# kfjahnke/envutil

Hardware: AMD Instinct MI355X
Metric: Mpix/s reprojected (16K lat/lon->cubemap, b-spline-3) (higher is better)
Workload: dtype f32

## Files before the change

### envutil_amd/csrc/eu_render4.hip

```cpp
#include <cstdio>
#include <cstring>
#include <vector>
#include <algorithm>
#include "eu_packed_dev.h"
#include "eu_launch.h"

#define EU4_TW 16
#define EU4_TH 8
#define EU4_WAVES 4
#ifndef EU4_WAVES0
#define EU4_WAVES0 1
#define EU4_TEXELS 384
#define EU4_OCC0 4
#endif
#define EU4_UNIT_ROWS 4
#define EU4_COL_FLOATS 8
#define EU4_MAX_PLANS 16

__device__ __forceinline__ void eu4_box_reduce(int &mn0, int &mn1, int &mx0, int &mx1)
{
#define EU4_RED(ctrl)                                        \
  "v_min_i32_dpp %0, %0, %0 " ctrl "\n\t"                    \
  "v_min_i32_dpp %1, %1, %1 " ctrl "\n\t"                    \
  "v_max_i32_dpp %2, %2, %2 " ctrl "\n\t"                    \
// ... 325 lines not shown
#pragma unroll 1
  for (int k = gid / EU4_SHARDS; k < nwork; k += (int)(gridDim.x * EU4_WAVES / EU4_SHARDS)) {
    const int id = __builtin_amdgcn_readfirstlane(p.wl[EU4_WL_ENTRIES + (size_t)k * EU4_SHARDS + sh]);
    const int tile_y = id / w.tiles16;
    const int x0 = (id - tile_y * w.tiles16) * EU4_TW;
    eu4_direct_tile<NCH, DEG, PRJ>(p, atab, tile_y, x0, lane);
  }
  __shared__ int last, listed;
  __syncthreads();
  if (threadIdx.x == 0) { listed = 0; last = atomicAdd(p.wl + EU4_WL_DONE1, 1) == (int)gridDim.x - 1; }
  __syncthreads();
  if (last) {
    int mine = 0;
    for (int i = threadIdx.x; i < EU4_SHARDS; i += 256)
      mine += __hip_atomic_load(p.wl + EU4_WL_SHARD(i), __ATOMIC_RELAXED, __HIP_MEMORY_SCOPE_AGENT);
    atomicAdd(&listed, mine);
    for (int i = threadIdx.x; i <= EU4_SHARDS + 8; i += 256)
      __hip_atomic_store(p.wl + 16 * i, 0, __ATOMIC_RELAXED, __HIP_MEMORY_SCOPE_AGENT);
    __syncthreads();
    if (threadIdx.x == 0) __hip_atomic_store(p.wl + EU4_WL_LISTED, listed, __ATOMIC_RELAXED, __HIP_MEMORY_SCOPE_AGENT);
  }
}

static long long eu4_followers_plan = 0, eu4_followers_last = 0;
extern "C" unsigned long long eu_hip_share_follower_tiles(void) { return (unsigned long long)eu4_followers_last; }
static int eu4_boxtab_last = 0;
static long long eu4_boxtab_tiles_last = 0;
extern "C" int eu_hip_boxtab_used(void) { return eu4_boxtab_last; }
extern "C" unsigned long long eu_hip_boxtab_tiles(void) { return (unsigned long long)eu4_boxtab_tiles_last; }

#ifndef EU4_DIRECT_WGS
#define EU4_DIRECT_WGS 2048
#endif

template <int NCH, int DEG, int PRJ>
static int launch4_ndp(const eu_render_params &p, const eu4_plan &w, hipStream_t st)
{
  if constexpr (PRJ == EU_SPHERICAL) {
    static const int cus = [] {
      int dev = 0, n = 0;
      if (hipGetDevice(&dev) != hipSuccess) return 0;
      if (hipDeviceGetAttribute(&n, hipDeviceAttributeMultiprocessorCount, dev) != hipSuccess) return 0;
      return n;
    }();
    const bool fast = eu_staged_fast_profile(p);
    const bool bt = fast && w.boxtab != nullptr && p.out_stride < (1ll << 25);
    int per_cu = 0;
    if (bt) {
      static const int occ = [] { int n = 0; return hipOccupancyMaxActiveBlocksPerMultiprocessor(&n, eu_render5_kernel<NCH, DEG, PRJ, true, true>, 64 * EU5_WAVES, 0) == hipSuccess ? n : 0; }();
      per_cu = occ;
    } else if (fast) {
      static const int occ = [] { int n = 0; return hipOccupancyMaxActiveBlocksPerMultiprocessor(&n, eu_render5_kernel<NCH, DEG, PRJ, true>, 64 * EU5_WAVES, 0) == hipSuccess ? n : 0; }();
      per_cu = occ;
    } else {
      static const int occ = [] { int n = 0; return hipOccupancyMaxActiveBlocksPerMultiprocessor(&n, eu_render5_kernel<NCH, DEG, PRJ, false>, 64 * EU5_WAVES, 0) == hipSuccess ? n : 0; }();
      per_cu = occ;
    }
    const int wgs = (cus / 8) * 8 * per_cu;
    if (wgs <= 0) return -1;
    if (fast) eu4_followers_last = eu4_followers_plan;
    eu4_boxtab_last = bt;
    if (bt) hipLaunchKernelGGL((eu_render5_kernel<NCH, DEG, PRJ, true, true>), dim3((unsigned)wgs), dim3(64 * EU5_WAVES), 0, st, p, w);
    else if (fast) hipLaunchKernelGGL((eu_render5_kernel<NCH, DEG, PRJ, true>), dim3((unsigned)wgs), dim3(64 * EU5_WAVES), 0, st, p, w);
    else hipLaunchKernelGGL((eu_render5_kernel<NCH, DEG, PRJ, false>), dim3((unsigned)wgs), dim3(64 * EU5_WAVES), 0, st, p, w);
  } else {
    const int units = (p.tiles_y + EU4_UNIT_ROWS - 1) / EU4_UNIT_ROWS;
    dim3 grid((unsigned)(8 * ((w.tiles16 + EU4_WAVES0 - 1) / EU4_WAVES0)), (unsigned)EU4_UNIT_ROWS, (unsigned)((units + 7) / 8));
    hipLaunchKernelGGL((eu_render4s_kernel<NCH, DEG, PRJ>), grid, dim3(64 * EU4_WAVES0), 0, st, p, w);
  }
  if (hipGetLastError() != hipSuccess) return -1;
  hipLaunchKernelGGL((eu_render4d_kernel<NCH, DEG, PRJ>), dim3(EU4_DIRECT_WGS), dim3(256), 0, st, p, w);
  if (hipGetLastError() != hipSuccess) {
    (void)hipMemsetAsync(p.wl, 0, EU4_WL_ENTRIES * sizeof(int), st);
    return -1;
  }
  return 0;
}

template <int NCH, int DEG>
static int launch4_nd(const eu_render_params &p, const eu4_plan &w, hipStream_t st)
{
  switch (p.src.prj) {
    case EU_SPHERICAL: return launch4_ndp<NCH, DEG, EU_SPHERICAL>(p, w, st);
    case EU_CUBEMAP: return launch4_ndp<NCH, DEG, EU_CUBEMAP>(p, w, st);
    case EU_BIATAN6: return launch4_ndp<NCH, DEG, EU_BIATAN6>(p, w, st);
  }
  return -2;
}

template <int NCH>
static int launch4_n(const eu_render_params &p, const eu4_plan &w, hipStream_t st)
{
  switch (p.src.degree) {
    case 1: return launch4_nd<NCH, 1>(p, w, st);
    case 2: return launch4_nd<NCH, 2>(p, w, st);
    case 3: return launch4_nd<NCH, 3>(p, w, st);
  }
  return -2;
}

static_assert(EU_STAGED_TILE_ROWS == EU4_TH && EU_STAGED_MAX_TILES_Y == 65535 * 8 * EU4_UNIT_ROWS, "eu_select.h: eu_staged_covers");
namespace {
struct plan_cache {
  std::vector<unsigned char> key;
  eu_dev_buf<int> tileplan, l2_rows, l1_ent, xtab, boxtab;
  bool has_boxtab = false;
  long long boxtab_tiles = 0;
  eu_dev_buf<float> coltab;
  float *atab = nullptr;
  int planned_rows = 0;
  int l2_off[9] = {};
  int l1_off[9] = {};
  int l1_ecols = 1;
  long long follower_tiles = 0;
  hipStream_t last_stream = nullptr;
} g4s[EU_MAX_SLOTS];
#define g4 (g4s[eu_current_slot()])

bool ensure_atab()
{
  if (g4.atab) return true;
  std::vector<float> tab(768, 0.0f);
  for (int i = 0; i < EU_ATAN_TAB_ENTRIES; i++) eu_atan_tab_entry(i, tab.data() + 8 * i);
  if (hipMalloc((void **)&g4.atab, tab.size() * sizeof(float)) != hipSuccess) return false;
  return hipMemcpy(g4.atab, tab.data(), tab.size() * sizeof(float), hipMemcpyHostToDevice) == hipSuccess;
}

template <int DEG>
void launch_colplan(const eu_render_params &p, float *ct, const float *k, hipStream_t st)
{
  hipLaunchKernelGGL((eu_colplan_kernel<DEG>), dim3((unsigned)((p.width + 511) / 512)), dim3(256), 0, st, p, ct,
                     k[0], k[1], k[2], k[3]);
}

std::vector<unsigned char> eu4_plan_key(const eu_render_params &p, unsigned long long plan_gen, const eu_switches &sw)
{
  std::vector<unsigned char> key(sizeof(unsigned long long) + sizeof(eu_src_dev) + 11 * sizeof(int));
  unsigned char *q = key.data();
  memcpy(q, &plan_gen, sizeof plan_gen); q += sizeof plan_gen;
  eu_src_dev sd = p.src; sd.base = nullptr;
  memcpy(q, &sd, sizeof sd); q += sizeof sd;
  const int v[11] = { p.width, p.row_begin, p.row_end, p.band_shift, p.band_count, p.band_index, p.form, p.norm_mode, sw.share,
                      sw.boxtab, sw.boxtab_max_kb };
  memcpy(q, v, sizeof v);
  return key;
}

bool upload(eu_dev_buf<int> &buf, const std::vector<int> &v, size_t spare)
{
  if (buf.reserve(v.size() + spare) != hipSuccess) return false;
  return v.empty() || hipMemcpy(buf.p, v.data(), v.size() * sizeof(int), hipMemcpyHostToDevice) == hipSuccess;
}

template <int DEG>
void launch_boxplan(const eu_render_params &p, const float *atab_g, const int *l2_rows, int tiles16, int ntiles, int *tab, hipStream_t st)
{
  hipLaunchKernelGGL((eu5_boxplan_kernel<DEG>), dim3((unsigned)((ntiles + 3) / 4)), dim3(256), 0, st, p, atab_g, l2_rows, tiles16,
                     ntiles, tab);
}

int eu4_build_plans(const eu_render_params &p, int tiles16, const eu_switches &sw, const float *h_row,
                    size_t h_row_floats, hipStream_t st)
{
  std::vector<int> tp((size_t)p.tiles_y, -1);
  std::vector<float> plans;
  const bool can = p.form == EU_FORM_BA && p.norm_mode == EU_NORM_NONE && h_row;
// ... 34 lines not shown
    for (int r = 0; r < p.tiles_y; r++)
      if (!paired(r >> 1)) rows[(r / EU5_UNIT_ROWS) & 7].push_back(r);
    for (int x = 0; x < 8; x++) { g4.l2_off[x] = (int)all.size(); all.insert(all.end(), rows[x].begin(), rows[x].end()); }
    g4.l2_off[8] = (int)all.size();
    if (!upload(g4.l2_rows, all, 1)) return -1;
  }
  g4.has_boxtab = false; g4.boxtab_tiles = 0;
  if (sw.boxtab && eu_staged_fast_profile(p)) {
    const long long ntiles = (long long)g4.l2_off[8] * tiles16;
    const long long bytes = ntiles * (EU5_BT_RECS * 16);
    if (bytes <= (long long)sw.boxtab_max_kb * 1024) {
      if (g4.boxtab.reserve((size_t)std::max<long long>(1, ntiles) * (EU5_BT_RECS * 4)) != hipSuccess) return -1;
      if (ntiles > 0) {
        switch (p.src.degree) {
          case 1: launch_boxplan<1>(p, g4.atab, g4.l2_rows.p, tiles16, (int)ntiles, g4.boxtab.p, st); break;
          case 2: launch_boxplan<2>(p, g4.atab, g4.l2_rows.p, tiles16, (int)ntiles, g4.boxtab.p, st); break;
          default: launch_boxplan<3>(p, g4.atab, g4.l2_rows.p, tiles16, (int)ntiles, g4.boxtab.p, st); break;
        }
        if (hipGetLastError() != hipSuccess) return -1;
      }
      g4.has_boxtab = true; g4.boxtab_tiles = ntiles;
    }
  }
  for (int j = 0; j < nplans; j++) {
    float *ct = g4.coltab.p + j * (size_t)p.width * EU4_COL_FLOATS;
    switch (p.src.degree) {
      case 1: launch_colplan<1>(p, ct, &plans[4 * j], st); break;
      case 2: launch_colplan<2>(p, ct, &plans[4 * j], st); break;
      default: launch_colplan<3>(p, ct, &plans[4 * j], st); break;
    }
    if (hipGetLastError() != hipSuccess) return -1;
  }
  std::vector<float> h_ct((size_t)nplans * p.width * EU4_COL_FLOATS);
  if (nplans) {
    if (hipStreamSynchronize(st) != hipSuccess) return -1;
    if (hipMemcpy(h_ct.data(), g4.coltab.p, h_ct.size() * sizeof(float), hipMemcpyDeviceToHost) != hipSuccess) return -1;
  }
  std::vector<int> cm, cp;
  for (int m = 0; 2 * m + 1 < p.tiles_y; m++)
    if (paired(m)) { cm.push_back(m); cp.push_back(tp[(size_t)2 * m]); }
  eu_share_input in;
  in.width = p.width; in.tiles16 = tiles16; in.row_begin = p.row_begin; in.row_end = p.row_end;
  in.band_mode = p.band_count > 1;
  in.ncand = (int)cm.size(); in.cand_m = cm.data(); in.cand_plan = cp.data();
  in.h_row = h_row; in.h_row_floats = h_row_floats; in.row_floats = EU_ROW_FLOATS;
  in.coltab = nplans ? h_ct.data() : nullptr; in.col_floats = EU4_COL_FLOATS; in.nplans = nplans;
// ... 5 lines not shown
  if (hipMemcpy(g4.xtab.p, gr.xtab.data(), gr.xtab.size() * sizeof(int), hipMemcpyHostToDevice) != hipSuccess) return -1;
  for (int x = 0; x < 9; x++) g4.l1_off[x] = gr.off[x];
  g4.l1_ecols = gr.ecols;
  g4.follower_tiles = gr.follower_tiles;
  return 0;
}

void eu4_fill_plan(eu4_plan &w)
{
  w.tileplan = g4.tileplan.p;
  w.coltab = g4.coltab.p;
  w.l2_rows = g4.l2_rows.p;
  for (int x = 0; x < 9; x++) w.l2_off[x] = g4.l2_off[x];
  w.l2_half = (w.tiles16 + 1) / 2;
  w.l2_magic = (1ull << 40) / (unsigned long long)w.l2_half + 1;
  w.l1_ent = g4.l1_ent.p;
  for (int x = 0; x < 9; x++) w.l1_off[x] = g4.l1_off[x];
  w.l1_ecols = g4.l1_ecols;
  w.l1_magic = (1ull << 40) / (unsigned long long)w.l1_ecols + 1;
  w.xtab = g4.xtab.p;
  w.boxtab = g4.has_boxtab ? g4.boxtab.p : nullptr;
}

int launch4(const eu_render_params &p, const eu4_plan &w, hipStream_t st)
{
  switch (p.nch) {
    case 3: return launch4_n<3>(p, w, st);
    case 4: return launch4_n<4>(p, w, st);
  }
  return -2;
}

#ifdef EU5_STAMPS
int launch4_stamped(const eu_render_params &p, eu4_plan &w, hipStream_t st)
{
  static unsigned long long *d_st = nullptr; static size_t st_cap = 0; static int dumps = 0;
  const size_t ntile_st = (size_t)w.tiles16 * p.tiles_y * 8;
  const size_t nst = ntile_st + 8192 * 4;
  if (st_cap < nst) { if (d_st) (void)hipFree(d_st); if (hipMalloc((void **)&d_st, nst * 8) != hipSuccess) return -1; st_cap = nst; }
  (void)hipMemsetAsync(d_st, 0, nst * 8, st);
  w.stamps = d_st;
  const int rc_ = launch4(p, w, st);
  if (rc_ == 0 && dumps < 2 && nst >= 8 * 4096) {
    dumps++;
    std::vector<unsigned long long> h(nst);
    (void)hipStreamSynchronize(st);
    (void)hipMemcpy(h.data(), d_st, nst * 8, hipMemcpyDeviceToHost);
    double acc[32][8] = {}; size_t cnt[32] = {};
    for (size_t t = 0; t < ntile_st / 8; t++) {
      const unsigned long long *q = &h[t * 8];
      if (!q[0] || !q[7]) continue;
      const int cls = (int)(q[1] & 31);
      cnt[cls]++;
      acc[cls][0] += (double)(q[2] - q[0]); acc[cls][1] += (double)(q[3] - q[2]);
      if (q[4]) { acc[cls][2] += (double)(q[4] - q[3]); acc[cls][3] += (double)(q[5] - q[4]); acc[cls][4] += (double)(q[6] - q[5]); }
      acc[cls][5] += (double)(q[7] - q[6]); acc[cls][6] += (double)(q[7] - q[0]);
    }
    {
      double mn = 1e30, mx = 0, sum = 0, l1 = 0, first = 1e30, last = 0; size_t nw = 0;
      for (size_t k = 0; k < 8192; k++) {
        const unsigned long long *q = &h[ntile_st + k * 4];
        if (!q[3]) continue;
        const double d = (double)(q[2] - q[0]);
        mn = std::min(mn, d); mx = std::max(mx, d); sum += d; l1 += (double)(q[1] - q[0]); nw++;
        first = std::min(first, (double)q[0]); last = std::max(last, (double)q[2]);
// ... 8 lines not shown
  return rc_;
}
#endif
}

extern "C" int eu_launch_render4(const eu_render_params *pp, const eu_switches *sw, const float *h_row, size_t h_row_floats,
                                 unsigned long long plan_gen, void *stream, int *launches)
{
  eu_render_params p = *pp;
  eu4_followers_last = 0;
  eu4_boxtab_last = 0; eu4_boxtab_tiles_last = 0;
  *launches = 2;
  if (!eu_staged_covers(p) || !p.wl) return -2;
  p.tiles_y = (p.row_end - p.row_begin + EU4_TH - 1) / EU4_TH;
  eu4_plan w;
  w.tiles16 = (p.width + EU4_TW - 1) / EU4_TW;
  if (w.tiles16 <= 0 || p.tiles_y <= 0) return 0;
  hipStream_t st = (hipStream_t)stream;
  if (!ensure_atab()) return -1;
  w.atab_g = g4.atab;
  if (p.src.prj == EU_SPHERICAL) {
    std::vector<unsigned char> key = eu4_plan_key(p, plan_gen, *sw);
    if (key != g4.key) {
      if (eu4_build_plans(p, w.tiles16, *sw, h_row, h_row_floats, st)) return -1;
      g4.key.swap(key);
    }
    if (sw->r4 != 1 && !eu_staged_worth(p.src.degree, g4.planned_rows, p.tiles_y)) { *launches = 0; return 0; }
  }
  eu4_fill_plan(w);
  eu4_followers_plan = g4.follower_tiles;
  eu4_boxtab_tiles_last = w.boxtab ? g4.boxtab_tiles : 0;
  g4.last_stream = st;
#ifdef EU5_STAMPS
  return launch4_stamped(p, w, st);
#else
  return launch4(p, w, st);
#endif
}
```

### envutil_amd/csrc/eu_render5.h

```cpp
#define EU5_WAVES 4
#ifndef EU5_TEXELS
#define EU5_TEXELS 576
#endif
#ifndef EU5_OCC
#define EU5_OCC 4
#endif
#ifndef EU5_UNIT_ROWS
#define EU5_UNIT_ROWS 4
#endif

typedef const __attribute__((address_space(3))) eu4_f4 *eu5_l4ptr;

template <int NCH, int DEG>
__device__ __forceinline__ void eu5_taps(eu_lptr lt, int a, int b, int pitch, const eu_f2 *wx, const eu_f2 *wy,
                                         eu_f2 tx, eu_f2 ty, eu_f2 &rga, eu_f2 &bxa, eu_f2 &rgb, eu_f2 &bxb)
{
  constexpr int order = DEG + 1;
  if constexpr (DEG == 1) {
    const eu_f2 wl0 = 1.0f - tx, wr0 = tx, wl1 = 1.0f - ty, wr1 = ty;
    const eu4_f4 a00 = *(eu5_l4ptr)(lt + a), a01 = *(eu5_l4ptr)(lt + a + 4);
    const eu4_f4 a10 = *(eu5_l4ptr)(lt + a + pitch), a11 = *(eu5_l4ptr)(lt + a + pitch + 4);
    const eu4_f4 b00 = *(eu5_l4ptr)(lt + b), b01 = *(eu5_l4ptr)(lt + b + 4);
    const eu4_f4 b10 = *(eu5_l4ptr)(lt + b + pitch), b11 = *(eu5_l4ptr)(lt + b + pitch + 4);
    {
// ... 566 lines not shown
  eu5_co8 c;
  eu5_coords8<DEG>(s, atab, T, c);
  eu5_split_y<DEG>(c);
  const eu_i2 hit = { va ? -1 : 0, vb ? -1 : 0 };
  eu5_boxes B;
  eu5_box_stage<DEG, true>(s.gate0, s.gate1, s.upper0, s.upper1, hit, c.ok, c.ixa, c.ixb, c.iya, c.iyb, B);
  const int cls = (B.npass < 0 || (B.npass > 0 && !B.clean)) ? EU5_BT_WORK : B.npass;
  eu5_box r[EU5_BT_RECS] = { B.full, B.full, B.full, B.full };
  if (B.npass == 2) { r[0] = eu5_box_at(B.h0, B.h1, B.h2, B.h3, 31); r[1] = eu5_box_at(B.h0, B.h1, B.h2, B.h3, 63); }
  if (B.npass == 4) {
#pragma unroll
    for (int k = 0; k < 4; k++) r[k] = eu5_box_at(B.q0, B.q1, B.q2, B.q3, 15 + 16 * k);
  }
  int v = 0;
#pragma unroll
  for (int k = 0; k < EU5_BT_RECS; k++) {
#pragma unroll
    for (int i = 0; i < 4; i++)
      if (lane == 4 * k + i) v = eu5_bt_pack(r[k], k == 0 ? cls : 0, i);
  }
  if (lane < 4 * EU5_BT_RECS) tab[(size_t)g * (4 * EU5_BT_RECS) + lane] = v;
}

template <int NCH, int DEG>
__device__ __forceinline__ void eu5_tile_bt(const eu_render_params &p, const eu4_plan &w, const float *atab, float *wtile,
                                            int tile_y, int x0, int lane, const eu5_tab8 &T, eu5_i4 R, eu5_crec rec,
                                            bool have_n, int ty_n, int x0_n, eu5_tab8 &Tn)
{
  constexpr int order = DEG + 1;
  const eu_src_dev &s = p.src;
#ifdef EU5_STAMPS
  unsigned long long st_[8] = { 0, 0, 0, 0, 0, 0, 0, 0 };
#endif
  EU5_STAMP(0);
  const int cls = R.w;
  if (cls & EU5_BT_WORK) {
    if (lane == 0) {
      const int id = tile_y * w.tiles16 + x0 / EU4_TW;
      const int sh = eu4_shard_of(id);
      const int slot = atomicAdd(p.wl + EU4_WL_SHARD(sh), 1);
      p.wl[EU4_WL_ENTRIES + (size_t)slot * EU4_SHARDS + sh] = id;
    }
    if (have_n) eu5_load8<true>(p, ty_n, x0_n, lane, Tn);
    __builtin_amdgcn_s_waitcnt(EU5_WAIT_VM0);
    return;
  }
  const int npass = cls & 7;
  const unsigned lds_tile = (unsigned)(unsigned long long)(eu4_lds_void)wtile;
  eu5_tab8 Tl = T;
  asm volatile("" : "+v"(Tl.c0), "+v"(Tl.A0), "+v"(Tl.A1), "+v"(Tl.A2), "+v"(Tl.B0), "+v"(Tl.B1), "+v"(Tl.B2));
  eu5_box bx = { R.x, R.y, R.x + (R.z & 0xffff), R.y + (R.z >> 16) };
  bool some = npass > 0 && R.z >= 0;
  if (some) eu5_stage<NCH, DEG>(s, bx, lds_tile, lane);
  const int pr = lane & 3, rw = (lane >> 2) & 7, hf = lane >> 5;
  const int y = p.row_begin + tile_y * EU4_TH + rw;
  const bool yin = y < p.row_end;
  const int xa = x0 + 8 * hf + 2 * pr, xb = xa + 1;
  const bool va = yin && xa < p.width, vb = yin && xb < p.width;
  eu_f2 rga = { 0.0f, 0.0f }, bxa = { 0.0f, 0.0f }, rgb = { 0.0f, 0.0f }, bxb = { 0.0f, 0.0f };
  if (npass > 0) {
    eu5_co8 c;
    eu5_coords8<DEG>(s, atab, Tl, c);
    eu5_split_y<DEG>(c);
#ifdef EU5_STAMPS
// ... 87 lines not shown
  const eu4_f4 *ea = (const eu4_f4 *)(ct + (size_t)xa * EU4_COL_FLOATS);
  const eu4_f4 *eb = (const eu4_f4 *)(ct + (size_t)xb * EU4_COL_FLOATS);
  T.a0 = ea[0]; T.a1 = ea[1]; T.b0 = eb[0]; T.b1 = eb[1];
}

__device__ __forceinline__ void eu5_y_reduce(int &mn, int &mx)
{
#define EU5_RED2(ctrl)                                       \
  "v_min_i32_dpp %0, %0, %0 " ctrl "\n\t"                    \
  "v_max_i32_dpp %1, %1, %1 " ctrl "\n\t"                    \
  "s_nop 1\n\t"
  asm("s_nop 1\n\t"
      EU5_RED2("row_shr:1 row_mask:0xf bank_mask:0xf")
      EU5_RED2("row_shr:2 row_mask:0xf bank_mask:0xf")
      EU5_RED2("row_shr:4 row_mask:0xf bank_mask:0xf")
      EU5_RED2("row_shr:8 row_mask:0xf bank_mask:0xf")
      EU5_RED2("row_bcast:15 row_mask:0xa bank_mask:0xf")
      EU5_RED2("row_bcast:31 row_mask:0xc bank_mask:0xf")
      : "+v"(mn), "+v"(mx));
#undef EU5_RED2
  mn = __builtin_amdgcn_readlane(mn, 63); mx = __builtin_amdgcn_readlane(mx, 63);
}

template <int NCH, int DEG>
__device__ __forceinline__ void eu5_group16(const eu_render_params &p, const eu4_plan &w, const float *atab, float *wtile,
                                            eu5_tab16 &T, eu5_cint ent, int n, int m0, int plan0, int tcol, int lane0,
                                            bool have_n, int m_n, int plan_n, int tcol_n)
{
  constexpr int order = DEG + 1;
  const eu_src_dev &s = p.src;
#ifdef EU5_STAMPS
  unsigned st_[8] = { 0, 0, 0, 0, 0, 0, 0, 0 };
#endif
  EU5_STAMP32(0);
  const eu5_cint xt = (eu5_cint)w.xtab;
  int xmn = xt[2 * (plan0 * w.tiles16 + tcol)], xmx = xt[2 * (plan0 * w.tiles16 + tcol) + 1];
  int iyAa, iyAb, iyBa, iyBb, bad, mny = INT_MAX, mxy = INT_MIN;
  eu_f2 tyA, tyB;
  bool off;
  {
    int lane = lane0;
    asm volatile("" : "+v"(lane));
    const int pr = lane & 3, rw = (lane >> 2) & 7, hf = lane >> 5;
    const int yA = p.row_begin + 2 * m0 * EU4_TH + rw, yB = yA + EU4_TH;
    const bool yinA = yA < p.row_end, yinB = yB < p.row_end;
    const int xa = tcol * EU4_TW + 8 * hf + 2 * pr, xb = xa + 1;
    const bool vxa = xa < p.width, vxb = xb < p.width;
// ... 75 lines not shown
      const int ixa = __float_as_int(T.a0.x), ixb = __float_as_int(T.b0.x);
      const eu_f2 tx = { T.a0.y, T.b0.y };
      if constexpr (DEG >= 2) {
        wx[0] = (eu_f2){ T.a0.z, T.b0.z }; wx[1] = (eu_f2){ T.a0.w, T.b0.w }; wx[2] = (eu_f2){ T.a1.x, T.b1.x };
        if constexpr (DEG == 3) wx[3] = (eu_f2){ T.a1.y, T.b1.y };
        eu_weights2<DEG>(s.wm, tyA, wyA); eu_weights2<DEG>(s.wm, tyB, wyB);
      }
      const int ibw = bx.mxx - bx.mnx + order;
      const int oAa = hAa ? ((iyAa - bx.mny) * ibw + (ixa - bx.mnx)) * 4 : 0, oAb = hAb ? ((iyAb - bx.mny) * ibw + (ixb - bx.mnx)) * 4 : 0;
      const int oBa = hBa ? ((iyBa - bx.mny) * ibw + (ixa - bx.mnx)) * 4 : 0, oBb = hBb ? ((iyBb - bx.mny) * ibw + (ixb - bx.mnx)) * 4 : 0;
      asm volatile("s_waitcnt vmcnt(0)" ::: "memory");
      __builtin_amdgcn_sched_barrier(0);
      eu5_taps<NCH, DEG>((eu_lptr)wtile, oAa, oAb, ibw * 4, wx, wyA, tx, tyA, rga, bxa, rgb, bxb);
      asm volatile("" : "+v"(rga), "+v"(bxa), "+v"(rgb), "+v"(bxb));
      {
        float qa[4] = { rga.x, rga.y, bxa.x, bxa.y }, qb[4] = { rgb.x, rgb.y, bxb.x, bxb.y };
        float *const orow = p.out + (long long)(ycA - p.row_begin) * p.out_stride;
        if (hAa) eu_put<NCH>(orow, xa, qa);
        if (hAb) eu_put<NCH>(orow, xb, qb);
      }
      __builtin_amdgcn_sched_barrier(0);
      eu5_taps<NCH, DEG>((eu_lptr)wtile, oBa, oBb, ibw * 4, wx, wyB, tx, tyB, rga, bxa, rgb, bxb);
      asm volatile("" : "+v"(rga), "+v"(bxa), "+v"(rgb), "+v"(bxb));
    } else if (mny != INT_MAX) {
      if (lane < 2) {
        const int id = (2 * mk + lane) * w.tiles16 + tc;
        const int sh = eu4_shard_of(id);
        const int slot = atomicAdd(p.wl + EU4_WL_SHARD(sh), 1);
        p.wl[EU4_WL_ENTRIES + (size_t)slot * EU4_SHARDS + sh] = id;
      }
    }
    if (k + 1 < n) {
      const int xa_n = mir_n ? p.width - 1 - (tcol * EU4_TW + xl) : tcol * EU4_TW + xl, xb_n = mir_n ? xa_n - 1 : xa_n + 1;
      const int xac = xa_n < p.width ? xa_n : p.width - 1, xbc = xb_n < p.width ? xb_n : p.width - 1;
      eu5_load_cols(w.coltab + (size_t)plan_k * p.width * EU4_COL_FLOATS, xac, xbc, T);
    } else if (have_n) {
      eu5_load16(p, w.coltab + (size_t)plan_n * p.width * EU4_COL_FLOATS, 2 * m_n, tcol_n * EU4_TW, lane, T);
    }
    __builtin_amdgcn_sched_barrier(0);
    if (fast) {
      float qa[4] = { rga.x, rga.y, bxa.x, bxa.y }, qb[4] = { rgb.x, rgb.y, bxb.x, bxb.y };
      float *const orow = p.out + (long long)(ycB - p.row_begin) * p.out_stride;
      if (hBa) eu_put<NCH>(orow, xa, qa);
      if (hBb) eu_put<NCH>(orow, xb, qb);
    }
    EU5_STAMP32(7);
#ifdef EU5_STAMPS
// ... 26 lines not shown
    rx += dx; ry += dy; ul += du;
    if (rx >= tiles16) { rx -= tiles16; ry++; }
    if (ry >= UNIT) { ry -= UNIT; ul++; }
  }
  __device__ __forceinline__ bool done() const { return ul * 8 + xcd >= units; }
  __device__ __forceinline__ int row() const { return (ul * 8 + xcd) * UNIT + ry; }
  __device__ __forceinline__ int col() const
  {
    const unsigned h = ((unsigned)row() * 0x9E3779B1u) >> 16;
    int c = rx + (int)((h * (unsigned)tiles16) >> 16);
    if (c >= tiles16) c -= tiles16;
    return c;
  }
};

__device__ __forceinline__ int eu5_pair_plan(const int *tileplan, int tiles_y, int m)
{
  if (2 * m + 1 >= tiles_y) return -1;
  const eu5_cint tp = (eu5_cint)tileplan;
  const int a = tp[2 * m], b = tp[2 * m + 1];
  return a == b ? a : -1;
}

template <int NCH, int DEG, int PRJ, bool FAST, bool BOXTAB = false>
__global__ __launch_bounds__(64 * EU5_WAVES, EU5_OCC) void eu_render5_kernel(const eu_render_params p, const eu4_plan w)
{
  __shared__ __attribute__((aligned(16))) float tile_all[EU5_WAVES * EU5_TEXELS * 4];
  __shared__ __attribute__((aligned(16))) float atab[768];
  const int lane0 = threadIdx.x & 63;
  const int wave = __builtin_amdgcn_readfirstlane(threadIdx.x >> 6);
  float *const tile = tile_all + wave * (EU5_TEXELS * 4);
  if (PRJ != EU_CUBEMAP && wave == 0) {
#pragma unroll
    for (int i = 0; i < 3; i++)
      __builtin_amdgcn_global_load_lds((eu4_gbl_void)(w.atab_g + i * 256 + lane0 * 4),
                                       (eu4_lds_void)(atab + i * 256), 16, 0, 0);
    asm volatile("s_waitcnt vmcnt(0)" ::: "memory");
  }
  __syncthreads();
#ifdef EU5_STAMPS
  const unsigned long long ws0 = __builtin_amdgcn_s_memtime();
  unsigned long long ws1 = ws0;
#endif
  const int xcd = (int)(blockIdx.x & 7);
  const int K = (int)(gridDim.x >> 3) * EU5_WAVES;
  const int t0 = (int)(blockIdx.x >> 3) * EU5_WAVES + wave;
  constexpr bool PAIRS = FAST && PRJ == EU_SPHERICAL;
  if constexpr (PAIRS) {
    const int n1 = (w.l1_off[xcd + 1] - w.l1_off[xcd]) * w.l1_ecols;
    const eu5_cint ents = (eu5_cint)w.l1_ent + EU_SHARE_ENTRY_INTS * w.l1_off[xcd];
    int pos1 = t0;
    auto seek = [&](eu5_cint &e, int &n, int &m, int &plan, int &tcol) -> bool {
      if (pos1 >= n1) return false;
      const int r = (int)(((unsigned long long)(unsigned)pos1 * w.l1_magic) >> 40);
      e = ents + EU_SHARE_ENTRY_INTS * r;
      n = e[0]; m = e[2]; plan = e[3];
      const unsigned h = ((unsigned)m * 0x9E3779B1u) >> 16;
      int c = pos1 - r * w.l1_ecols + (int)((h * (unsigned)w.l1_ecols) >> 16);
      if (c >= w.l1_ecols) c -= w.l1_ecols;
      tcol = e[1] + c;
      pos1 += K;
      return true;
    };
    eu5_cint e_a = ents, e_n = ents;
    int n_a = 0, m_a = 0, col_a = 0, plan_a = 0, n_n = 0, m_n = 0, col_n = 0, plan_n = 0;
    bool have_a = seek(e_a, n_a, m_a, plan_a, col_a);
    eu5_tab16 T;
    if (have_a) eu5_load16(p, w.coltab + (size_t)plan_a * p.width * EU4_COL_FLOATS, 2 * m_a, col_a * EU4_TW, lane0, T);
#pragma unroll 1
    while (have_a) {
      const bool have_n = seek(e_n, n_n, m_n, plan_n, col_n);
      eu5_group16<NCH, DEG>(p, w, atab, tile, T, e_a, n_a, m_a, plan_a, col_a, lane0, have_n, m_n, have_n ? plan_n : 0, col_n);
      e_a = e_n; n_a = n_n; m_a = m_n; plan_a = plan_n; col_a = col_n; have_a = have_n;
    }
  }
#ifdef EU5_STAMPS
  ws1 = __builtin_amdgcn_s_memtime();
#endif
  eu5_iter<EU5_UNIT_ROWS> it;
  it.xcd = xcd; it.tiles16 = w.tiles16;
  it.units = (p.tiles_y + EU5_UNIT_ROWS - 1) / EU5_UNIT_ROWS;
  it.start(t0, K);
  if constexpr (PAIRS) {
    int *const queue = p.wl + EU4_WL_DYN(xcd);
    const int nbatch = (w.l2_off[xcd + 1] - w.l2_off[xcd]) * w.l2_half;
    const eu5_cint rows2 = (eu5_cint)w.l2_rows + w.l2_off[xcd];
    auto take = [&]() -> int {
      int v = 0;
      if (lane0 == 0) v = atomicAdd(queue, 1);
      return v;
    };
    if constexpr (BOXTAB) {
      static_assert(FAST && PRJ == EU_SPHERICAL, "the box table is that of the FAST lat/lon second loop");
      const eu5_crec bt = (eu5_crec)w.boxtab;
      auto decode = [&](int j, int &ty, int &tcol, int &ti) -> bool {
        if (j >= nbatch) return false;
        const int r = (int)(((unsigned long long)(unsigned)j * w.l2_magic) >> 40);
        ty = rows2[r]; tcol = 2 * (j - r * w.l2_half);
        ti = ((w.l2_off[xcd] + r) * w.tiles16 + tcol) * EU5_BT_RECS;
        return true;
      };
      int ty_a = 0, col_a = 0, ti_a = 0, ty_n = 0, col_n = 0, ti_n = 0;
      bool have = decode(__builtin_amdgcn_readfirstlane(take()), ty_a, col_a, ti_a);
      eu5_tab8 Ta, Tb;
      eu5_i4 Ra = { 0, 0, -1, 0 }, Rb = { 0, 0, -1, 0 };
      if (have) { Ra = bt[ti_a]; eu5_load8<FAST>(p, ty_a, col_a * EU4_TW, lane0, Ta); }
      __builtin_amdgcn_s_waitcnt(EU5_WAIT_VM0);
#pragma unroll 1
      while (have) {
        const int jn_lane = take();
        const bool second = col_a + 1 < w.tiles16;
        if (second) Rb = bt[ti_a + EU5_BT_RECS];
        {
          int lane = lane0;
          asm volatile("" : "+v"(lane));
          eu5_tile_bt<NCH, DEG>(p, w, atab, tile, ty_a, col_a * EU4_TW, lane, Ta, Ra, bt + ti_a, second, ty_a,
                                (col_a + 1) * EU4_TW, Tb);
        }
        const bool have_n = decode(__builtin_amdgcn_readfirstlane(jn_lane), ty_n, col_n, ti_n);
        if (have_n) Ra = bt[ti_n];
        if (second) {
          int lane = lane0;
          asm volatile("" : "+v"(lane));
          eu5_tile_bt<NCH, DEG>(p, w, atab, tile, ty_a, (col_a + 1) * EU4_TW, lane, Tb, Rb, bt + ti_a + EU5_BT_RECS, have_n,
                                ty_n, col_n * EU4_TW, Ta);
        } else if (have_n) {
          eu5_load8<FAST>(p, ty_n, col_n * EU4_TW, lane0, Ta);
          __builtin_amdgcn_s_waitcnt(EU5_WAIT_VM0);
        }
        ty_a = ty_n; col_a = col_n; ti_a = ti_n; have = have_n;
      }
    } else {
      auto decode = [&](int j, int &ty, int &tcol) -> bool {
        if (j >= nbatch) return false;
        const int r = (int)(((unsigned long long)(unsigned)j * w.l2_magic) >> 40);
        ty = rows2[r]; tcol = 2 * (j - r * w.l2_half);
        return true;
      };
      int ty_a = 0, col_a = 0, ty_n = 0, col_n = 0;
      bool have = decode(__builtin_amdgcn_readfirstlane(take()), ty_a, col_a);
      eu5_tab8 Ta, Tb;
      if (have) eu5_load8<FAST>(p, ty_a, col_a * EU4_TW, lane0, Ta);
  #pragma unroll 1
      while (have) {
        const int jn_lane = take();
        const bool second = col_a + 1 < w.tiles16;
        {
// ... 41 lines not shown
```

### envutil_amd/csrc/eu_select.h

```cpp
#ifndef EU_SELECT_H
#define EU_SELECT_H
#include <algorithm>
#include <climits>
#include <cstdlib>
#include <vector>
#include "eu_device.h"
#include "eu_share_groups.h"
#include "eu_worklist.h"

struct eu_switches {
  int force_general;
  int hybrid;
  int r4;
  int colmajor;
  int rej;
  int colplan;
  int share;
  int direct;
  int iir_stream;
  int boxtab;
  int boxtab_max_kb;
  int views_max_kb;
};

#define EU_BOXTAB_MAX_KB 65536
#define EU_VIEWS_MAX_KB 65536

inline eu_switches eu_read_switches()
{
  auto first = [](const char *name) { const char *e = getenv(name); return e ? e[0] : '\0'; };
  eu_switches s;
  s.force_general = first("EU_HIP_KERNEL") == '1';
  const char hy = first("EU_HIP_HYBRID");
  s.hybrid = hy == '0' ? 0 : hy == '2' ? 2 : 1;
  const char *r4 = getenv("EU_HIP_R4");
  s.r4 = r4 ? atoi(r4) : -1;
  const char *cm = getenv("EU_HIP_COLMAJOR");
  s.colmajor = cm && cm[0] ? atoi(cm) : -1;
  const char rj = first("EU_HIP_REJ");
  s.rej = rj == '1' ? 1 : rj == '2' ? 2 : 0;
  s.colplan = first("EU_HIP_COLPLAN") != '0';
  const char sh = first("EU_HIP_SHARE");
  s.share = sh == '0' ? 0 : sh == 'm' ? EU_SHARE_MIRRORS : sh == 'f' ? EU_SHARE_FACES : EU_SHARE_FACES | EU_SHARE_MIRRORS;
  s.direct = first("EU_HIP_DIRECT") == '1';
  const char *iir = getenv("EU_HIP_IIR_STREAM");
  s.iir_stream = iir ? atoi(iir) : 7;
  s.boxtab = first("EU_HIP_BOXTAB") != '0';
  const char *bm = getenv("EU_HIP_BOXTAB_MAX_KB");
  s.boxtab_max_kb = bm && bm[0] ? std::max(0, std::min(atoi(bm), 16 * 1024 * 1024)) : EU_BOXTAB_MAX_KB;
  const char *vm = getenv("EU_HIP_VIEWS_MAX_KB");
  s.views_max_kb = vm && vm[0] ? std::max(0, std::min(atoi(vm), 16 * 1024 * 1024)) : EU_VIEWS_MAX_KB;
  return s;
}

inline bool eu_cube_source(int prj) { return prj == EU_CUBEMAP || prj == EU_BIATAN6; }

inline bool eu_packed_covers_source(const eu_src_dev &s, int nch, int nch_out)
{
  if (s.has_lcp || nch_out != nch) return false;
  if (s.prj != EU_SPHERICAL && !eu_cube_source(s.prj)) return false;
  if (s.degree < 1 || s.degree > 3 || s.es0 != nch) return false;
  return nch >= 1 && nch <= 4;
}
inline bool eu_packed_covers(const eu_render_params &p)
{
  if (p.stage != 0 || p.form >= EU_FORM_FISH) return false;
  return eu_packed_covers_source(p.src, p.nch, p.nch_out);
}

#define EU_STAGED_TILE_ROWS 8
#define EU_STAGED_TILE_COLS 16
#define EU_STAGED_MAX_TILES_Y (65535 * 8 * 4)
inline unsigned long long eu_staged_tiles(int width, int row_begin, int row_end)
{
// ... 110 lines not shown
```

### envutil_amd/csrc/eu_worklist.h

```cpp
#ifndef EU_WORKLIST_H
#define EU_WORKLIST_H
#include <algorithm>
#include <climits>
#include <cstddef>
#include <vector>

#if defined(__HIPCC__)
#define EU_WL_FN __host__ __device__ inline __attribute__((always_inline))
#else
#define EU_WL_FN inline
#endif

#define EU4_SHARDS 1024
#define EU4_WL_SHARD(s) (16 * (s))
#define EU4_WL_DONE1 (16 * EU4_SHARDS)
#define EU4_WL_DYN(x) (16 * (EU4_SHARDS + 1 + (x)))
#define EU4_WL_LISTED (16 * (EU4_SHARDS + 9))
#define EU4_WL_ENTRIES (16 * (EU4_SHARDS + 16))

#define EU4_WL_MAX_TILES ((size_t)INT_MAX)

EU_WL_FN int eu4_shard_of(int id)
{
  return (int)(((unsigned)id * 0x9E3779B1u) >> 22) & (EU4_SHARDS - 1);
}

class eu4_wl_census {
  std::vector<unsigned> count_;
  std::vector<size_t> grows_;
  size_t n_ = 0;
  unsigned fullest_ = 0;

public:
  eu4_wl_census() : count_(EU4_SHARDS, 0u) {}
  size_t fullest(size_t ntiles)
  {
    for (; n_ < ntiles; n_++) {
      const unsigned c = ++count_[(size_t)eu4_shard_of((int)n_)];
      if (c > fullest_) { fullest_ = c; grows_.push_back(n_ + 1); }
    }
    return (size_t)(std::upper_bound(grows_.begin(), grows_.end(), ntiles) - grows_.begin());
  }
};

inline size_t eu_render4_worklist_header_ints(void) { return EU4_WL_ENTRIES; }

inline size_t eu_render4_worklist_ints(size_t ntiles)
{
  static eu4_wl_census census;
  if (ntiles > EU4_WL_MAX_TILES) return 0;
  return EU4_WL_ENTRIES + census.fullest(ntiles) * EU4_SHARDS;
}

#endif
```

Baseline: 110,200.

## Record direct-tile list once and replay it on later renders

On the first render with an unchanged plan, a single-block kernel turns the sharded worklist into a deduplicated, compacted tile list via a bitmap and prefix scan. Later renders launch a replay variant of the main kernel that skips the atomic worklist appends. They then run a new list-driven direct kernel that strides over the recorded tiles instead of scanning shards. This removes per-frame atomics and shard scanning, but relies on the set of direct tiles depending only on geometry, and it adds plan-cache state and extra memory.

```diff
diff --git a/envutil_amd/csrc/eu_render4.hip b/envutil_amd/csrc/eu_render4.hip
--- a/envutil_amd/csrc/eu_render4.hip
+++ b/envutil_amd/csrc/eu_render4.hip
@@ -371,6 +371,85 @@
   }
 }
 
+static_assert(EU4_SHARDS == 1024, "eu4_dlist_compact_kernel: one thread per shard");
+__global__ __launch_bounds__(1024) void eu4_dlist_compact_kernel(const int *wl, unsigned *bits, int ntiles, int *dl)
+{
+  __shared__ int sc[1024];
+  const int t = threadIdx.x;
+  const int m = wl[EU4_WL_SHARD(t)];
+  for (int k = 0; k < m; k++) {
+    const int id = wl[EU4_WL_ENTRIES + (size_t)k * EU4_SHARDS + t];
+    if ((unsigned)id < (unsigned)ntiles) atomicOr(bits + (id >> 5), 1u << (id & 31));
+  }
+  __threadfence();
+  __syncthreads();
+  const int nwords = (int)(((long long)ntiles + 31) / 32);
+  const int per = (nwords + 1023) / 1024;
+  const int a = min(t * per, nwords), b = min(a + per, nwords);
+  int cnt = 0;
+  for (int i = a; i < b; i++) cnt += __popc(__hip_atomic_load(bits + i, __ATOMIC_RELAXED, __HIP_MEMORY_SCOPE_AGENT));
+  sc[t] = cnt;
+  __syncthreads();
+  for (int d = 1; d < 1024; d <<= 1) {
+    const int v = t >= d ? sc[t - d] : 0;
+    __syncthreads();
+    sc[t] += v;
+    __syncthreads();
+  }
+  int o = sc[t] - cnt;
+  for (int i = a; i < b; i++) {
+    unsigned word = __hip_atomic_load(bits + i, __ATOMIC_RELAXED, __HIP_MEMORY_SCOPE_AGENT);
+    for (; word; word &= word - 1) dl[EU4_DL_ENTRIES + (size_t)o++] = i * 32 + (__ffs((int)word) - 1);
+  }
+  if (t == 1023) dl[EU4_DL_COUNT] = sc[1023];
+}
+
+template <int NCH, int DEG, int PRJ>
+__global__ __launch_bounds__(256, 4) void eu_render4l_kernel(const eu_render_params p, const eu4_plan w, const int *dl)
+{
+  __shared__ __attribute__((aligned(16))) float atab[768];
+  const int lane = threadIdx.x & 63;
+  const int wave = __builtin_amdgcn_readfirstlane(threadIdx.x >> 6);
+  if (wave == 0) {
+#pragma unroll
+    for (int i = 0; i < 3; i++)
+      __builtin_amdgcn_global_load_lds((eu4_gbl_void)(w.atab_g + i * 256 + lane * 4), (eu4_lds_void)(atab + i * 256), 16, 0, 0);
+    asm volatile("s_waitcnt vmcnt(0)" ::: "memory");
+  }
+  const int n = __builtin_amdgcn_readfirstlane(dl[EU4_DL_COUNT]);
+  __syncthreads();
+  const int g = (int)blockIdx.x * EU4_WAVES + wave, W = (int)gridDim.x * EU4_WAVES;
+  const int mine = eu4_dl_take(n, g, W);
+#pragma unroll 1
+  for (int i = 0; i < mine; i++) {
+    const int id = __builtin_amdgcn_readfirstlane(dl[EU4_DL_ENTRIES + (size_t)eu4_dl_index(g, i, W)]);
+    const int tile_y = id / w.tiles16;
+    const int x0 = (id - tile_y * w.tiles16) * EU4_TW;
+    eu4_direct_tile<NCH, DEG, PRJ>(p, atab, tile_y, x0, lane);
+  }
+  __shared__ int last;
+  __syncthreads();
+  if (threadIdx.x == 0) last = atomicAdd(p.wl + EU4_WL_DONE1, 1) == (int)gridDim.x - 1;
+  __syncthreads();
+  if (last) {
+    if (threadIdx.x <= 8) __hip_atomic_store(p.wl + 16 * (EU4_SHARDS + threadIdx.x), 0, __ATOMIC_RELAXED, __HIP_MEMORY_SCOPE_AGENT);
+    if (threadIdx.x == 0) __hip_atomic_store(p.wl + EU4_WL_LISTED, n, __ATOMIC_RELAXED, __HIP_MEMORY_SCOPE_AGENT);
+  }
+}
+
+enum { EU4_DL_OFF, EU4_DL_RECORD, EU4_DL_REPLAY };
+struct eu4_dlist {
+  int mode;
+  int *dl;
+  unsigned *bits;
+  int ntiles;
+};
+
+static bool eu4_boxtab_form(const eu_render_params &p, const eu4_plan &w)
+{
+  return eu_staged_fast_profile(p) && w.boxtab != nullptr && p.out_stride < (1ll << 25);
+}
+
 static long long eu4_followers_plan = 0, eu4_followers_last = 0;
 extern "C" unsigned long long eu_hip_share_follower_tiles(void) { return (unsigned long long)eu4_followers_last; }
 static int eu4_boxtab_last = 0;
@@ -383,8 +462,9 @@
 #endif
 
 template <int NCH, int DEG, int PRJ>
-static int launch4_ndp(const eu_render_params &p, const eu4_plan &w, hipStream_t st)
-{
+static int launch4_ndp(const eu_render_params &p, const eu4_plan &w, const eu4_dlist &d, hipStream_t st)
+{
+  int mode = EU4_DL_OFF;
   if constexpr (PRJ == EU_SPHERICAL) {
     static const int cus = [] {
       int dev = 0, n = 0;
@@ -393,9 +473,13 @@
       return n;
     }();
     const bool fast = eu_staged_fast_profile(p);
-    const bool bt = fast && w.boxtab != nullptr && p.out_stride < (1ll << 25);
+    const bool bt = eu4_boxtab_form(p, w);
+    if (bt) mode = d.mode;
     int per_cu = 0;
-    if (bt) {
+    if (mode == EU4_DL_REPLAY) {
+      static const int occ = [] { int n = 0; return hipOccupancyMaxActiveBlocksPerMultiprocessor(&n, eu_render5_kernel<NCH, DEG, PRJ, true, true, false>, 64 * EU5_WAVES, 0) == hipSuccess ? n : 0; }();
+      per_cu = occ;
+    } else if (bt) {
       static const int occ = [] { int n = 0; return hipOccupancyMaxActiveBlocksPerMultiprocessor(&n, eu_render5_kernel<NCH, DEG, PRJ, true, true>, 64 * EU5_WAVES, 0) == hipSuccess ? n : 0; }();
       per_cu = occ;
     } else if (fast) {
@@ -409,7 +493,8 @@
     if (wgs <= 0) return -1;
     if (fast) eu4_followers_last = eu4_followers_plan;
     eu4_boxtab_last = bt;
-    if (bt) hipLaunchKernelGGL((eu_render5_kernel<NCH, DEG, PRJ, true, true>), dim3((unsigned)wgs), dim3(64 * EU5_WAVES), 0, st, p, w);
+    if (mode == EU4_DL_REPLAY) hipLaunchKernelGGL((eu_render5_kernel<NCH, DEG, PRJ, true, true, false>), dim3((unsigned)wgs), dim3(64 * EU5_WAVES), 0, st, p, w);
+    else if (bt) hipLaunchKernelGGL((eu_render5_kernel<NCH, DEG, PRJ, true, true>), dim3((unsigned)wgs), dim3(64 * EU5_WAVES), 0, st, p, w);
     else if (fast) hipLaunchKernelGGL((eu_render5_kernel<NCH, DEG, PRJ, true>), dim3((unsigned)wgs), dim3(64 * EU5_WAVES), 0, st, p, w);
     else hipLaunchKernelGGL((eu_render5_kernel<NCH, DEG, PRJ, false>), dim3((unsigned)wgs), dim3(64 * EU5_WAVES), 0, st, p, w);
   } else {
@@ -418,6 +503,34 @@
     hipLaunchKernelGGL((eu_render4s_kernel<NCH, DEG, PRJ>), grid, dim3(64 * EU4_WAVES0), 0, st, p, w);
   }
   if (hipGetLastError() != hipSuccess) return -1;
+  if constexpr (PRJ == EU_SPHERICAL) {
+    if (mode == EU4_DL_REPLAY) {
+      static const int wgs = [] {
+        int dev = 0, cus = 0, n = 0;
+        if (hipGetDevice(&dev) != hipSuccess) return 0;
+        if (hipDeviceGetAttribute(&cus, hipDeviceAttributeMultiprocessorCount, dev) != hipSuccess) return 0;
+        if (hipOccupancyMaxActiveBlocksPerMultiprocessor(&n, eu_render4l_kernel<NCH, DEG, PRJ>, 64 * EU4_WAVES, 0) != hipSuccess) return 0;
+        return cus * n;
+      }();
+      if (wgs > 0) hipLaunchKernelGGL((eu_render4l_kernel<NCH, DEG, PRJ>), dim3((unsigned)wgs), dim3(64 * EU4_WAVES), 0, st, p, w, (const int *)d.dl);
+      if (wgs <= 0 || hipGetLastError() != hipSuccess) {
+        (void)hipMemsetAsync(p.wl, 0, EU4_WL_ENTRIES * sizeof(int), st);
+        return -1;
+      }
+      return 0;
+    }
+    if (mode == EU4_DL_RECORD) {
+      bool ok = hipMemsetAsync(d.bits, 0, eu_render4_dlist_bitmap_ints((size_t)d.ntiles) * sizeof(int), st) == hipSuccess;
+      if (ok) {
+        hipLaunchKernelGGL(eu4_dlist_compact_kernel, dim3(1), dim3(1024), 0, st, (const int *)p.wl, d.bits, d.ntiles, d.dl);
+        ok = hipGetLastError() == hipSuccess;
+      }
+      if (!ok) {
+        (void)hipMemsetAsync(p.wl, 0, EU4_WL_ENTRIES * sizeof(int), st);
+        return -1;
+      }
+    }
+  }
   hipLaunchKernelGGL((eu_render4d_kernel<NCH, DEG, PRJ>), dim3(EU4_DIRECT_WGS), dim3(256), 0, st, p, w);
   if (hipGetLastError() != hipSuccess) {
     (void)hipMemsetAsync(p.wl, 0, EU4_WL_ENTRIES * sizeof(int), st);
@@ -427,23 +540,23 @@
 }
 
 template <int NCH, int DEG>
-static int launch4_nd(const eu_render_params &p, const eu4_plan &w, hipStream_t st)
+static int launch4_nd(const eu_render_params &p, const eu4_plan &w, const eu4_dlist &d, hipStream_t st)
 {
   switch (p.src.prj) {
-    case EU_SPHERICAL: return launch4_ndp<NCH, DEG, EU_SPHERICAL>(p, w, st);
-    case EU_CUBEMAP: return launch4_ndp<NCH, DEG, EU_CUBEMAP>(p, w, st);
-    case EU_BIATAN6: return launch4_ndp<NCH, DEG, EU_BIATAN6>(p, w, st);
+    case EU_SPHERICAL: return launch4_ndp<NCH, DEG, EU_SPHERICAL>(p, w, d, st);
+    case EU_CUBEMAP: return launch4_ndp<NCH, DEG, EU_CUBEMAP>(p, w, d, st);
+    case EU_BIATAN6: return launch4_ndp<NCH, DEG, EU_BIATAN6>(p, w, d, st);
   }
   return -2;
 }
 
 template <int NCH>
-static int launch4_n(const eu_render_params &p, const eu4_plan &w, hipStream_t st)
+static int launch4_n(const eu_render_params &p, const eu4_plan &w, const eu4_dlist &d, hipStream_t st)
 {
   switch (p.src.degree) {
-    case 1: return launch4_nd<NCH, 1>(p, w, st);
-    case 2: return launch4_nd<NCH, 2>(p, w, st);
-    case 3: return launch4_nd<NCH, 3>(p, w, st);
+    case 1: return launch4_nd<NCH, 1>(p, w, d, st);
+    case 2: return launch4_nd<NCH, 2>(p, w, d, st);
+    case 3: return launch4_nd<NCH, 3>(p, w, d, st);
   }
   return -2;
 }
@@ -455,6 +568,9 @@
   eu_dev_buf<int> tileplan, l2_rows, l1_ent, xtab, boxtab;
   bool has_boxtab = false;
   long long boxtab_tiles = 0;
+  eu_dev_buf<int> dlist;
+  eu_dev_buf<unsigned> dlbits;
+  bool has_dlist = false, dlist_recorded = false;
   eu_dev_buf<float> coltab;
   float *atab = nullptr;
   int planned_rows = 0;
@@ -484,13 +600,13 @@
 
 std::vector<unsigned char> eu4_plan_key(const eu_render_params &p, unsigned long long plan_gen, const eu_switches &sw)
 {
-  std::vector<unsigned char> key(sizeof(unsigned long long) + sizeof(eu_src_dev) + 11 * sizeof(int));
+  std::vector<unsigned char> key(sizeof(unsigned long long) + sizeof(eu_src_dev) + 12 * sizeof(int));
   unsigned char *q = key.data();
   memcpy(q, &plan_gen, sizeof plan_gen); q += sizeof plan_gen;
   eu_src_dev sd = p.src; sd.base = nullptr;
   memcpy(q, &sd, sizeof sd); q += sizeof sd;
-  const int v[11] = { p.width, p.row_begin, p.row_end, p.band_shift, p.band_count, p.band_index, p.form, p.norm_mode, sw.share,
-                      sw.boxtab, sw.boxtab_max_kb };
+  const int v[12] = { p.width, p.row_begin, p.row_end, p.band_shift, p.band_count, p.band_index, p.form, p.norm_mode, sw.share,
+                      sw.boxtab, sw.boxtab_max_kb, sw.dlist };
   memcpy(q, v, sizeof v);
   return key;
 }
@@ -571,6 +687,15 @@
       g4.has_boxtab = true; g4.boxtab_tiles = ntiles;
     }
   }
+  g4.has_dlist = false; g4.dlist_recorded = false;
+  if (sw.dlist && g4.has_boxtab) {
+    const size_t all = (size_t)tiles16 * (size_t)p.tiles_y;
+    if ((eu_render4_dlist_ints(all) + eu_render4_dlist_bitmap_ints(all)) * sizeof(int) <= (size_t)sw.boxtab_max_kb * 1024) {
+      if (g4.dlist.reserve(eu_render4_dlist_ints(all)) != hipSuccess) return -1;
+      if (g4.dlbits.reserve(eu_render4_dlist_bitmap_ints(all)) != hipSuccess) return -1;
+      g4.has_dlist = true;
+    }
+  }
   for (int j = 0; j < nplans; j++) {
     float *ct = g4.coltab.p + j * (size_t)p.width * EU4_COL_FLOATS;
     switch (p.src.degree) {
@@ -622,17 +747,17 @@
   w.boxtab = g4.has_boxtab ? g4.boxtab.p : nullptr;
 }
 
-int launch4(const eu_render_params &p, const eu4_plan &w, hipStream_t st)
+int launch4(const eu_render_params &p, const eu4_plan &w, const eu4_dlist &d, hipStream_t st)
 {
   switch (p.nch) {
-    case 3: return launch4_n<3>(p, w, st);
-    case 4: return launch4_n<4>(p, w, st);
+    case 3: return launch4_n<3>(p, w, d, st);
+    case 4: return launch4_n<4>(p, w, d, st);
   }
   return -2;
 }
 
 #ifdef EU5_STAMPS
-int launch4_stamped(const eu_render_params &p, eu4_plan &w, hipStream_t st)
+int launch4_stamped(const eu_render_params &p, eu4_plan &w, const eu4_dlist &d, hipStream_t st)
 {
   static unsigned long long *d_st = nullptr; static size_t st_cap = 0; static int dumps = 0;
   const size_t ntile_st = (size_t)w.tiles16 * p.tiles_y * 8;
@@ -640,7 +765,7 @@
   if (st_cap < nst) { if (d_st) (void)hipFree(d_st); if (hipMalloc((void **)&d_st, nst * 8) != hipSuccess) return -1; st_cap = nst; }
   (void)hipMemsetAsync(d_st, 0, nst * 8, st);
   w.stamps = d_st;
-  const int rc_ = launch4(p, w, st);
+  const int rc_ = launch4(p, w, d, st);
   if (rc_ == 0 && dumps < 2 && nst >= 8 * 4096) {
     dumps++;
     std::vector<unsigned long long> h(nst);
@@ -695,6 +820,7 @@
   if (p.src.prj == EU_SPHERICAL) {
     std::vector<unsigned char> key = eu4_plan_key(p, plan_gen, *sw);
     if (key != g4.key) {
+      g4.has_dlist = false; g4.dlist_recorded = false;
       if (eu4_build_plans(p, w.tiles16, *sw, h_row, h_row_floats, st)) return -1;
       g4.key.swap(key);
     }
@@ -704,9 +830,21 @@
   eu4_followers_plan = g4.follower_tiles;
   eu4_boxtab_tiles_last = w.boxtab ? g4.boxtab_tiles : 0;
   g4.last_stream = st;
+  eu4_dlist d = { EU4_DL_OFF, nullptr, nullptr, 0 };
+  if (p.src.prj == EU_SPHERICAL && g4.has_dlist && eu4_boxtab_form(p, w)) {
+    d.dl = g4.dlist.p; d.bits = g4.dlbits.p; d.ntiles = w.tiles16 * p.tiles_y;
+    if (g4.dlist_recorded) d.mode = EU4_DL_REPLAY;
+    else {
+      hipStreamCaptureStatus cs = hipStreamCaptureStatusActive;
+      if (hipStreamIsCapturing(st, &cs) == hipSuccess && cs == hipStreamCaptureStatusNone) d.mode = EU4_DL_RECORD;
+      else (void)hipGetLastError();
+    }
+  }
 #ifdef EU5_STAMPS
-  return launch4_stamped(p, w, st);
+  const int rc = launch4_stamped(p, w, d, st);
 #else
-  return launch4(p, w, st);
+  const int rc = launch4(p, w, d, st);
 #endif
-}
+  if (rc == 0 && d.mode == EU4_DL_RECORD) g4.dlist_recorded = true;
+  return rc;
+}
diff --git a/envutil_amd/csrc/eu_render5.h b/envutil_amd/csrc/eu_render5.h
--- a/envutil_amd/csrc/eu_render5.h
+++ b/envutil_amd/csrc/eu_render5.h
@@ -612,7 +612,7 @@
   if (lane < 4 * EU5_BT_RECS) tab[(size_t)g * (4 * EU5_BT_RECS) + lane] = v;
 }
 
-template <int NCH, int DEG>
+template <int NCH, int DEG, bool APPEND = true>
 __device__ __forceinline__ void eu5_tile_bt(const eu_render_params &p, const eu4_plan &w, const float *atab, float *wtile,
                                             int tile_y, int x0, int lane, const eu5_tab8 &T, eu5_i4 R, eu5_crec rec,
                                             bool have_n, int ty_n, int x0_n, eu5_tab8 &Tn)
@@ -625,11 +625,13 @@
   EU5_STAMP(0);
   const int cls = R.w;
   if (cls & EU5_BT_WORK) {
-    if (lane == 0) {
-      const int id = tile_y * w.tiles16 + x0 / EU4_TW;
-      const int sh = eu4_shard_of(id);
-      const int slot = atomicAdd(p.wl + EU4_WL_SHARD(sh), 1);
-      p.wl[EU4_WL_ENTRIES + (size_t)slot * EU4_SHARDS + sh] = id;
+    if constexpr (APPEND) {
+      if (lane == 0) {
+        const int id = tile_y * w.tiles16 + x0 / EU4_TW;
+        const int sh = eu4_shard_of(id);
+        const int slot = atomicAdd(p.wl + EU4_WL_SHARD(sh), 1);
+        p.wl[EU4_WL_ENTRIES + (size_t)slot * EU4_SHARDS + sh] = id;
+      }
     }
     if (have_n) eu5_load8<true>(p, ty_n, x0_n, lane, Tn);
     __builtin_amdgcn_s_waitcnt(EU5_WAIT_VM0);
@@ -763,7 +765,7 @@
   mn = __builtin_amdgcn_readlane(mn, 63); mx = __builtin_amdgcn_readlane(mx, 63);
 }
 
-template <int NCH, int DEG>
+template <int NCH, int DEG, bool APPEND = true>
 __device__ __forceinline__ void eu5_group16(const eu_render_params &p, const eu4_plan &w, const float *atab, float *wtile,
                                             eu5_tab16 &T, eu5_cint ent, int n, int m0, int plan0, int tcol, int lane0,
                                             bool have_n, int m_n, int plan_n, int tcol_n)
@@ -885,7 +887,7 @@
       __builtin_amdgcn_sched_barrier(0);
       eu5_taps<NCH, DEG>((eu_lptr)wtile, oBa, oBb, ibw * 4, wx, wyB, tx, tyB, rga, bxa, rgb, bxb);
       asm volatile("" : "+v"(rga), "+v"(bxa), "+v"(rgb), "+v"(bxb));
-    } else if (mny != INT_MAX) {
+    } else if (APPEND && mny != INT_MAX) {
       if (lane < 2) {
         const int id = (2 * mk + lane) * w.tiles16 + tc;
         const int sh = eu4_shard_of(id);
@@ -958,11 +960,12 @@
   return a == b ? a : -1;
 }
 
-template <int NCH, int DEG, int PRJ, bool FAST, bool BOXTAB = false>
+template <int NCH, int DEG, int PRJ, bool FAST, bool BOXTAB = false, bool APPEND = true>
 __global__ __launch_bounds__(64 * EU5_WAVES, EU5_OCC) void eu_render5_kernel(const eu_render_params p, const eu4_plan w)
 {
   __shared__ __attribute__((aligned(16))) float tile_all[EU5_WAVES * EU5_TEXELS * 4];
   __shared__ __attribute__((aligned(16))) float atab[768];
+  static_assert(APPEND || BOXTAB, "only the box-table form has a replay instantiation");
   const int lane0 = threadIdx.x & 63;
   const int wave = __builtin_amdgcn_readfirstlane(threadIdx.x >> 6);
   float *const tile = tile_all + wave * (EU5_TEXELS * 4);
@@ -1006,7 +1009,7 @@
 #pragma unroll 1
     while (have_a) {
       const bool have_n = seek(e_n, n_n, m_n, plan_n, col_n);
-      eu5_group16<NCH, DEG>(p, w, atab, tile, T, e_a, n_a, m_a, plan_a, col_a, lane0, have_n, m_n, have_n ? plan_n : 0, col_n);
+      eu5_group16<NCH, DEG, APPEND>(p, w, atab, tile, T, e_a, n_a, m_a, plan_a, col_a, lane0, have_n, m_n, have_n ? plan_n : 0, col_n);
       e_a = e_n; n_a = n_n; m_a = m_n; plan_a = plan_n; col_a = col_n; have_a = have_n;
     }
   }
@@ -1050,7 +1053,7 @@
         {
           int lane = lane0;
           asm volatile("" : "+v"(lane));
-          eu5_tile_bt<NCH, DEG>(p, w, atab, tile, ty_a, col_a * EU4_TW, lane, Ta, Ra, bt + ti_a, second, ty_a,
+          eu5_tile_bt<NCH, DEG, APPEND>(p, w, atab, tile, ty_a, col_a * EU4_TW, lane, Ta, Ra, bt + ti_a, second, ty_a,
                                 (col_a + 1) * EU4_TW, Tb);
         }
         const bool have_n = decode(__builtin_amdgcn_readfirstlane(jn_lane), ty_n, col_n, ti_n);
@@ -1058,7 +1061,7 @@
         if (second) {
           int lane = lane0;
           asm volatile("" : "+v"(lane));
-          eu5_tile_bt<NCH, DEG>(p, w, atab, tile, ty_a, (col_a + 1) * EU4_TW, lane, Tb, Rb, bt + ti_a + EU5_BT_RECS, have_n,
+          eu5_tile_bt<NCH, DEG, APPEND>(p, w, atab, tile, ty_a, (col_a + 1) * EU4_TW, lane, Tb, Rb, bt + ti_a + EU5_BT_RECS, have_n,
                                 ty_n, col_n * EU4_TW, Ta);
         } else if (have_n) {
           eu5_load8<FAST>(p, ty_n, col_n * EU4_TW, lane0, Ta);
diff --git a/envutil_amd/csrc/eu_select.h b/envutil_amd/csrc/eu_select.h
--- a/envutil_amd/csrc/eu_select.h
+++ b/envutil_amd/csrc/eu_select.h
@@ -21,6 +21,7 @@
   int boxtab;
   int boxtab_max_kb;
   int views_max_kb;
+  int dlist;
 };
 
 #define EU_BOXTAB_MAX_KB 65536
@@ -50,6 +51,7 @@
   s.boxtab_max_kb = bm && bm[0] ? std::max(0, std::min(atoi(bm), 16 * 1024 * 1024)) : EU_BOXTAB_MAX_KB;
   const char *vm = getenv("EU_HIP_VIEWS_MAX_KB");
   s.views_max_kb = vm && vm[0] ? std::max(0, std::min(atoi(vm), 16 * 1024 * 1024)) : EU_VIEWS_MAX_KB;
+  s.dlist = first("EU_HIP_DLIST") != '0';
   return s;
 }
 
diff --git a/envutil_amd/csrc/eu_worklist.h b/envutil_amd/csrc/eu_worklist.h
--- a/envutil_amd/csrc/eu_worklist.h
+++ b/envutil_amd/csrc/eu_worklist.h
@@ -43,6 +43,14 @@
   }
 };
 
+#define EU4_DL_COUNT 0
+#define EU4_DL_ENTRIES 16
+inline size_t eu_render4_dlist_ints(size_t ntiles) { return EU4_DL_ENTRIES + ntiles; }
+inline size_t eu_render4_dlist_bitmap_ints(size_t ntiles) { return (ntiles + 31) / 32; }
+
+EU_WL_FN int eu4_dl_take(int n, int g, int W) { return g < n ? (n - g - 1) / W + 1 : 0; }
+EU_WL_FN int eu4_dl_index(int g, int i, int W) { return g + i * W; }
+
 inline size_t eu_render4_worklist_header_ints(void) { return EU4_WL_ENTRIES; }
 
 inline size_t eu_render4_worklist_ints(size_t ntiles)
```

After: 111,000, median of 4. About the same (+0.7%).
